# ShittyWizard/DiplomJourney

Hardware: AMD Instinct MI355X
Metric: candidate N-step rollouts/sec + MPC-step p50 latency, 1/2/4/8 MI355X (higher is better)
Workload: dtype f64

## Files before the change

diplomjourney_amd/csrc/mpc_device.h:

```cpp
#pragma once

#include <hip/hip_runtime.h>
#include <stdint.h>

#include "../../include/mpc_rollout.h"
#include "mpc_trig.h"

namespace mpc {

struct Consts {
  double x, y, phi;
  double x_t, y_t;
  double x_0, y_0;
  double A, B, C1, C2;
  double inv_den;
  double L, inv_L;
  double h;
  double hlgth;
  double s0, c0;
  int32_t L_pow2;
  int32_t pad_;
};

MPC_HD __forceinline__ Consts consts_from_problem(const mpc_problem_t& p) {
  Consts K;
  K.x = p.x;
  K.y = p.y;
  K.phi = p.phi;
  K.x_t = p.x_t;
  K.y_t = p.y_t;
  K.x_0 = p.x_0;
  K.y_0 = p.y_0;
  K.A = p.y_t - p.y_0;
  K.B = p.x_t - p.x_0;
  K.C1 = p.x_t * p.y_0;
  K.C2 = p.y_t * p.x_0;
  K.inv_den = 1.0 / sqrt(K.A * K.A + K.B * K.B);
  K.L = p.L;
  int e;
  const double m = frexp(p.L, &e);
  K.L_pow2 = (m == 0.5) ? 1 : 0;
  K.inv_L = K.L_pow2 ? 1.0 / p.L : 0.0;
  K.h = p.t_b - p.t_a;
  K.hlgth = 0.5 * (p.t_b - p.t_a);
  trig::sincos_fast(p.phi, &K.s0, &K.c0);
  K.pad_ = 0;
  return K;
}

constexpr double kWGK[11] = {
    0.011694638867371874278064396062192, 0.032558162307964727478818972459390,
    0.054755896574351996031381300244580, 0.075039674810919952767043140916190,
    0.093125454583697605535065465083366, 0.109387158802297641899210590325805,
    0.123491976262065851077208698889469, 0.134709217311473325928054001771707,
    0.142775938577060080797094273138717, 0.147739104901338491374841515972068,
    0.149445554002916905664936468389821};

template <int INTEG>
MPC_HD __forceinline__ double quad_const(double f, const Consts& K) {
  if constexpr (INTEG == MPC_INTEG_RECT) {
    return f * K.h;
  } else {
    double resk = kWGK[10] * f;
    const double fsum = f + f;
#pragma unroll
    for (int j = 1; j <= 9; j += 2) resk = resk + kWGK[j] * fsum;
#pragma unroll
    for (int j = 0; j <= 8; j += 2) resk = resk + kWGK[j] * fsum;
    return resk * K.hlgth;
  }
}

template <int INTEG>
MPC_HD __forceinline__ double heading_incr(double w, double t, const Consts& K) {
  if constexpr (INTEG == MPC_INTEG_RECT)
    return (w * K.h) * t;
  else
    return quad_const<INTEG>(w * t, K);
}

template <int INTEG>
MPC_HD __forceinline__ double position_step(double p, double v, double trig, const Consts& K) {
  if constexpr (INTEG == MPC_INTEG_RECT)
    return fma(v * K.h, trig, p);
  else
    return p + quad_const<INTEG>(v * trig, K);
}

constexpr int kRotCum = 2;

template <int INTEG, int ROT, bool PL2>
MPC_HD __forceinline__ void step_core(double& x, double& y, double& ph, double& s, double& c,
                                      double v, double beta, const Consts& K, bool& bad,
                                      const trig::Leads* ld = nullptr) {
  bad |= !(fabs(beta) <= trig::kTanMax);
  const double t = trig::tan_small(beta, ld);
  double dphi, vh = 0.0;
  if constexpr (PL2 && INTEG == MPC_INTEG_RECT && ROT == kRotCum) {
    vh = v * (K.h * K.inv_L);
    dphi = vh * t;
  } else if constexpr (PL2 && INTEG == MPC_INTEG_RECT) {
    vh = v * K.h;
    dphi = (vh * K.inv_L) * t;
  } else {
    const double w = PL2 ? v * K.inv_L : v / K.L;
    dphi = heading_incr<INTEG>(w, t, K);
  }
  ph = ph + dphi;
  if constexpr (ROT) {
    bad |= !(fabs(dphi) <= trig::kRotMax);
    double sd, cd;
    trig::rotation_sc(dphi, sd, cd, ld);
    trig::rotate_sc(sd, cd, s, c);
  } else {
    bad |= !(fabs(ph) <= trig::kFastMax);
    trig::sincos_core(ph, &s, &c);
  }
  if constexpr (PL2 && INTEG == MPC_INTEG_RECT) {
    x = fma(vh, c, x);
    y = fma(vh, s, y);
  } else {
    x = position_step<INTEG>(x, v, c, K);
    y = position_step<INTEG>(y, v, s, K);
  }
}

template <int ROT>
MPC_HD __forceinline__ void step_start(const Consts& K, double& x, double& y, double& ph,
                                       double& s, double& c) {
  ph = K.phi;
  if constexpr (ROT == kRotCum) {
    x = 0.0;
    y = 0.0;
    s = 0.0;
    c = 1.0;
  } else {
    x = K.x;
    y = K.y;
    s = K.s0;
    c = K.c0;
  }
}

template <bool SCALED>
MPC_HD __forceinline__ void cum_pose(const Consts& K, double A, double B, double& x, double& y) {
  if constexpr (SCALED) {
    A = A * K.L;
    B = B * K.L;
  }
  x = K.x + fma(K.c0, A, -(K.s0 * B));
  y = K.y + fma(K.s0, A, K.c0 * B);
}

template <int INTEG>
MPC_HD __forceinline__ void step_safe(double& x, double& y, double& ph, double v, double beta,
                                      const Consts& K) {
  const double w = K.L_pow2 ? v * K.inv_L : v / K.L;
  const double dphi = heading_incr<INTEG>(w, trig::tan_fast(beta), K);
  ph = ph + dphi;
  double s, c;
  trig::sincos_fast(ph, &s, &c);
  x = position_step<INTEG>(x, v, c, K);
  y = position_step<INTEG>(y, v, s, K);
}

MPC_HD __forceinline__ double crit_sqrt(double x) {
#if defined(__HIP_DEVICE_COMPILE__)
  const double y = __builtin_amdgcn_rsq(fmax(x, 0x1p-767));
  double g = x * y, h = y * 0.5;
  const double r = fma(-h, g, 0.5);
  g = fma(g, r, g);
  h = fma(h, r, h);
  double d = fma(-g, g, x);
  g = fma(d, h, g);
  d = fma(-g, g, x);
  return fma(d, h, g);
#else
  return sqrt(x);
#endif
}

MPC_HD __forceinline__ double cost(double x, double y, const Consts& K) {
  const double ex = K.x_t - x, ey = K.y_t - y;
  const double dist_target = crit_sqrt(ex * ex + ey * ey);
  const double dl = fabs(K.A * x - K.B * y + K.C1 - K.C2) * K.inv_den;
  const double d = (x == K.x_0 && y == K.y_0) ? 1000.0 : dl;
  return 10000.0 * dist_target + 10000.0 * (d * d);
}

struct Circle {
  double cx, cy, r2, pad_;
};
struct Obstacles {
  Circle c[MPC_MAX_OBSTACLES];
};
struct ObstacleArgs {
  Obstacles loop, world;
};
#if defined(__HIP_DEVICE_COMPILE__)
typedef const __attribute__((address_space(4))) Obstacles* ObsTable;
#else
typedef const Obstacles* ObsTable;
#endif

struct NoObs {
  static constexpr bool kOn = false;
};

template <int NOBS>
struct CircleObs {
  static_assert(NOBS >= 1 && NOBS <= MPC_MAX_OBSTACLES, "circle count");
  static constexpr bool kOn = true;
  ObsTable loop_t, world_t;
  template <int CPL>
  __device__ __forceinline__ static void test(ObsTable t, const double (&x)[CPL],
                                              const double (&y)[CPL], bool (&blocked)[CPL]) {
#if defined(__HIP_DEVICE_COMPILE__)
    if constexpr (NOBS > 4) asm volatile("" : "+s"(t));
#endif
#pragma unroll
    for (int i = 0; i < NOBS; ++i) {
      const double cx = t->c[i].cx, cy = t->c[i].cy, r2 = t->c[i].r2;
#pragma unroll
      for (int j = 0; j < CPL; ++j) {
        const double dx = x[j] - cx, dy = y[j] - cy;
        blocked[j] |= fma(dy, dy, dx * dx) < r2;
      }
    }
  }
  template <int CPL>
  __device__ __forceinline__ void loop(const double (&x)[CPL], const double (&y)[CPL],
                                       bool (&blocked)[CPL]) const {
    test<CPL>(loop_t, x, y, blocked);
  }
  __device__ __forceinline__ void world(double x, double y, bool& blocked) const {
    const double xs[1] = {x}, ys[1] = {y};
    bool bl[1] = {blocked};
    test<1>(world_t, xs, ys, bl);
    blocked = bl[0];
  }
};

MPC_HD __forceinline__ Circle frame_circle(const Consts& K, const Circle& w, bool scaled) {
  const double sc = scaled ? K.inv_L : 1.0;
  const double dx = w.cx - K.x, dy = w.cy - K.y;
  return Circle{(K.c0 * dx + K.s0 * dy) * sc, (K.c0 * dy - K.s0 * dx) * sc, w.r2 * (sc * sc), 0.0};
}

template <int INTEG, int ROT, bool PL2>
MPC_HD inline double rollout_candidate_l(const Consts& K, const double* v, const double* b,
                                         int64_t ld, int64_t col, int n_steps, double* traj) {
  double x, y, ph, s, c;
  step_start<ROT>(K, x, y, ph, s, c);
  bool bad = false;
  for (int st = 0; st < n_steps; ++st) {
    step_core<INTEG, ROT, PL2>(x, y, ph, s, c, v[st * ld + col], b[st * ld + col], K, bad);
    if (traj) {
      if constexpr (ROT == kRotCum) {
        cum_pose<PL2>(K, x, y, traj[3 * st + 0], traj[3 * st + 1]);
      } else {
        traj[3 * st + 0] = x;
        traj[3 * st + 1] = y;
      }
      traj[3 * st + 2] = ph;
    }
  }
  if constexpr (ROT == kRotCum) {
    if (!bad) cum_pose<PL2>(K, x, y, x, y);
  }
  if (bad) {
    x = K.x;
    y = K.y;
    ph = K.phi;
    for (int st = 0; st < n_steps; ++st) {
      step_safe<INTEG>(x, y, ph, v[st * ld + col], b[st * ld + col], K);
      if (traj) {
        traj[3 * st + 0] = x;
        traj[3 * st + 1] = y;
        traj[3 * st + 2] = ph;
      }
    }
  }
  return cost(x, y, K);
}

template <int INTEG, int ROT>
MPC_HD inline double rollout_candidate(const Consts& K, const double* v, const double* b,
                                       int64_t ld, int64_t col, int n_steps, double* traj) {
  return K.L_pow2 ? rollout_candidate_l<INTEG, ROT, true>(K, v, b, ld, col, n_steps, traj)
                  : rollout_candidate_l<INTEG, ROT, false>(K, v, b, ld, col, n_steps, traj);
}

}
```

diplomjourney_amd/csrc/mpc_generated.h:

```cpp
#pragma once

#include <hip/hip_runtime.h>
#include <stdint.h>

#include "mpc_argmin.h"
#include "mpc_device.h"
#include "mpc_episode.h"
#include "mpc_sampler.h"

namespace mpc {

__device__ inline void episode_grids(const mpc_episode_config_t& c, const EpisodeHead& S,
                                     double* s_v, double* s_b, int& nv_out, int& nb_out) {
  const int lane = threadIdx.x & 63;
  const uint64_t below = (lane == 0) ? 0ull : (~0ull >> (64 - lane));
  const int n_v = 1 + 2 * static_cast<int>(c.ratio_v);
  int nv = 0;
  double vmin = __builtin_inf();
  for (int base = 0; base < n_v; base += 64) {
    const int i = base + lane;
    const double cand = S.v + c.delta_v * (static_cast<double>(i) - c.ratio_v);
    const bool ok = i < n_v && !(cand < 0.0) && cand < c.v_max;
    const uint64_t m = __ballot(ok);
    const int pos = nv + __popcll(m & below);
    if (ok && pos < kEpMaxGrid) s_v[pos] = cand;
    if (S.steps_for_slowing > 0) {
      double mn = ok ? cand : __builtin_inf();
      for (int off = 32; off > 0; off >>= 1) mn = fmin(mn, __shfl_xor(mn, off, 64));
      vmin = fmin(vmin, mn);
    }
    nv += __popcll(m);
  }
  nv = nv < kEpMaxGrid ? nv : kEpMaxGrid;
  if (S.steps_for_slowing > 0 && nv > 0) {
    const double vel = vmin > c.v_min ? vmin : c.v_min;
    for (int i = lane; i < nv; i += 64) s_v[i] = vel;
  }
  const int n_b = 1 + 2 * static_cast<int>(c.ratio_beta);
  int nb = 0;
  for (int base = 0; base < n_b; base += 64) {
    const int i = base + lane;
    const double cand = S.beta + c.delta_beta * (static_cast<double>(i) - c.ratio_beta);
    const bool ok = i < n_b && fabs(cand) <= c.beta_bound;
    const uint64_t m = __ballot(ok);
    const int pos = nb + __popcll(m & below);
    if (ok && pos < kEpMaxGrid) s_b[pos] = cand;
    nb += __popcll(m);
  }
  nv_out = nv;
  nb_out = nb < kEpMaxGrid ? nb : kEpMaxGrid;
}

#ifndef MPC_TEMPLATES_ONLY
__global__ __launch_bounds__(kBlock) void k_episode_sample(
    mpc_episode_config_t c, EpisodeState* __restrict__ S, int64_t n_cand, int n_steps,
    int64_t base, double* __restrict__ v, double* __restrict__ b, int pairs) {
  __shared__ double s_v[kEpMaxGrid], s_b[kEpMaxGrid];
  __shared__ double2 s_grid[kSampleLdsEntries];
  __shared__ int s_nv, s_nb;
  if (threadIdx.x < 64) {
    int nv, nb;
    episode_grids(c, S->h, s_v, s_b, nv, nb);
    if (threadIdx.x == 0) {
      s_nv = nv;
      s_nb = nb;
    }
  }
  __syncthreads();
  const int nv = s_nv, nb = s_nb;
  const uint64_t seed = S->h.seed;
  const uint32_t n_grid = static_cast<uint32_t>(nv) * static_cast<uint32_t>(nb);
  const bool staged = n_grid <= static_cast<uint32_t>(kSampleLdsEntries);
  if (staged)
    for (uint32_t k = threadIdx.x; k < n_grid; k += kBlock)
      s_grid[k] = make_double2(s_v[k / nb], s_b[k % nb]);
  __syncthreads();
  if (blockIdx.x == 0 && threadIdx.x == 0) {
    S->h.nv = nv;
    S->h.nb = nb;
    for (int i = 0; i < nv; ++i) S->grid_v[i] = s_v[i];
    for (int i = 0; i < nb; ++i) S->grid_b[i] = s_b[i];
  }
  if (n_grid == 0 && !c.enumerate) return;
  if (!staged) {
    for (int64_t cc = blockIdx.x * static_cast<int64_t>(kBlock) + threadIdx.x; cc < n_cand;
         cc += static_cast<int64_t>(gridDim.x) * kBlock) {
      const uint64_t g = static_cast<uint64_t>(base + cc);
      for (int st = 0; st < n_steps; ++st) {
        const bool pad = c.enumerate && g >= n_grid;
        const uint32_t k = pad ? 0u : grid_entry(seed, st, g, n_grid, 1);
        v[ctl_off<false>(st, cc, n_cand)] = pad ? __builtin_nan("") : s_v[k / nb];
        b[ctl_off<false>(st, cc, n_cand)] = pad ? 0.0 : s_b[k % nb];
      }
    }
    return;
  }
  sample_items(s_grid, n_grid, n_cand, n_steps, seed, base, c.enumerate ? 2 : 1, v, b, n_cand,
               pairs);
}
#endif

template <int INTEG, int ROT, bool PL2>
__device__ __forceinline__ void generated_lane(const Consts& K, const double2* s_grid,
                                               uint32_t n_grid, uint64_t seed, uint64_t g0,
                                               int n_steps, double (&cst)[2]) {
  double x[2], y[2], ph[2], sn[2], cs[2];
  bool bad[2];
#pragma unroll
  for (int j = 0; j < 2; ++j) {
    step_start<ROT>(K, x[j], y[j], ph[j], sn[j], cs[j]);
    bad[j] = false;
  }
  trig::Leads lead = trig::const_leads();
#pragma unroll 1
  for (int st = 0; st < n_steps; ++st) {
    const double2 e0 = s_grid[grid_entry(seed, st, g0, n_grid, 1)];
    const double2 e1 = s_grid[grid_entry(seed, st, g0 + 1, n_grid, 1)];
    double ph0 = ROT ? 0.0 : ph[0], ph1 = ROT ? 0.0 : ph[1];
    step_core<INTEG, ROT, PL2>(x[0], y[0], ph0, sn[0], cs[0], e0.x, e0.y, K, bad[0], &lead);
    step_core<INTEG, ROT, PL2>(x[1], y[1], ph1, sn[1], cs[1], e1.x, e1.y, K, bad[1], &lead);
    if (!ROT) {
      ph[0] = ph0;
      ph[1] = ph1;
    }
  }
  if constexpr (ROT == kRotCum) {
#pragma unroll
    for (int j = 0; j < 2; ++j)
      if (!bad[j]) cum_pose<PL2>(K, x[j], y[j], x[j], y[j]);
  }
#pragma unroll
  for (int j = 0; j < 2; ++j) {
    if (bad[j]) {
      x[j] = K.x;
      y[j] = K.y;
      ph[j] = K.phi;
      for (int sr = 0; sr < n_steps; ++sr) {
        const double2 e = s_grid[grid_entry(seed, sr, g0 + j, n_grid, 1)];
        step_safe<INTEG>(x[j], y[j], ph[j], e.x, e.y, K);
      }
    }
    cst[j] = cost(x[j], y[j], K);
  }
}

constexpr int kGenWaves = 4;
template <int INTEG, int ROT, bool PL2>
__global__ __launch_bounds__(kBlock, kGenWaves) void k_rollout_generated(
    mpc_episode_config_t c, EpisodeState* __restrict__ S, int64_t n_cand, int n_steps,
    int64_t base, Rec* __restrict__ part, double* __restrict__ part_v,
    double* __restrict__ part_b) {
  extern __shared__ double2 s_gen_grid[];
  __shared__ double s_v[kEpMaxGrid], s_b[kEpMaxGrid];
  __shared__ int s_nv, s_nb;
  if (threadIdx.x < 64) {
    int nv, nb;
    episode_grids(c, S->h, s_v, s_b, nv, nb);
    if (threadIdx.x == 0) {
      s_nv = nv;
      s_nb = nb;
    }
  }
  __syncthreads();
  const int nv = s_nv, nb = s_nb;
  const uint32_t n_grid = static_cast<uint32_t>(nv) * static_cast<uint32_t>(nb);
  for (uint32_t k = threadIdx.x; k < n_grid; k += kBlock)
    s_gen_grid[k] = make_double2(s_v[k / nb], s_b[k % nb]);
  if (blockIdx.x == 0 && threadIdx.x == 0) {
    if ((S->h.K.L_pow2 != 0) != PL2) S->chain_error = 2u;
    S->h.nv = nv;
    S->h.nb = nb;
    for (int i = 0; i < nv; ++i) S->grid_v[i] = s_v[i];
    for (int i = 0; i < nb; ++i) S->grid_b[i] = s_b[i];
  }
  __syncthreads();
  const uint64_t seed = S->h.seed;
  const Consts K = S->h.K;
  const int64_t n_tiles = (n_cand + kBlock * 2 - 1) / (kBlock * 2);
  uint64_t best_k = ~0ull;
  int64_t best_i = INT64_MAX;
  if (n_grid > 0) {
    for (int64_t tile = blockIdx.x; tile < n_tiles; tile += gridDim.x) {
      const int64_t c0 = tile * (kBlock * 2) + threadIdx.x * 2;
      if (c0 < n_cand) {
        double cst[2];
        const uint64_t g0 = static_cast<uint64_t>(base + c0);
        generated_lane<INTEG, ROT, PL2>(K, s_gen_grid, n_grid, seed, g0, n_steps, cst);
#pragma unroll
        for (int j = 0; j < 2; ++j) {
          const uint64_t kk = cost_key_nonneg(cst[j]);
          if (kk < best_k) {
            best_k = kk;
            best_i = c0 + j;
          }
        }
      }
    }
  }
  block_argmin(best_k, best_i);
  if (threadIdx.x == 0) part[blockIdx.x] = Rec{best_k, best_i};
  __shared__ int64_t s_best;
  if (threadIdx.x == 0) s_best = best_k == ~0ull ? -1 : best_i;
  __syncthreads();
  const int64_t bi = s_best;
  if (bi >= 0 && threadIdx.x < n_steps) {
    const double2 e =
        s_gen_grid[grid_entry(seed, threadIdx.x, static_cast<uint64_t>(base + bi), n_grid, 1)];
    part_v[blockIdx.x * MPC_MAX_STEPS + threadIdx.x] = e.x;
    part_b[blockIdx.x * MPC_MAX_STEPS + threadIdx.x] = e.y;
  }
}

}
```

diplomjourney_amd/csrc/mpc_rollout.hip:

```cpp
#include <hip/hip_ext.h>
#include <hip/hip_runtime.h>

#include <math.h>
#include <stdint.h>
#include <string.h>

#include <algorithm>
#include <mutex>
#include <type_traits>

#include "../../include/mpc_rollout.h"
#include "mpc_argmin.h"
#include "mpc_chain.h"
#include "mpc_comm.h"
#include "mpc_device.h"
#include "mpc_dispatch.h"
#include "mpc_episode.h"
#include "mpc_episode_obs.h"
#include "mpc_episodes.h"
#include "mpc_episodes_obs_launch.h"
#include "mpc_exchange.h"
#include "mpc_finalize.h"
#include "mpc_ftepisodes.h"
#include "mpc_fulltree.h"
// ... 378 lines not shown
      k_episodes_run<I, R><<<n_robots, kBlock, 0, st>>>(dcfg, robots, n_steps, max_calls, log, cap,
                                                        progress);
    });
  else
    launch_episodes_run_obs(st, integrator, world_obstacles(obstacles, n_obstacles), n_obstacles,
                            n_robots, dcfg, robots, n_steps, max_calls, log, cap, progress,
                            n_blocked_out);
  return last_hip_status();
}

}
}

using namespace mpc;

extern "C" {

const char* mpc_version(void) { return "diplomjourney_amd mpc_rollout 0.2 (gfx950)"; }

const char* mpc_strerror(int status) {
  switch (status) {
    case MPC_OK: return "ok";
    case MPC_ERR_ARG: return "invalid argument";
    case MPC_ERR_WORKSPACE: return "workspace too small";
    case MPC_ERR_HIP: return "HIP runtime error";
    case MPC_ERR_UNSUPPORTED: return "unsupported option";
    default: return "unknown status";
  }
}

size_t mpc_workspace_bytes(int64_t n_cand, int32_t n_steps) {
  (void)n_steps;
  if (n_cand < 0) return 0;
  return static_cast<size_t>(rollout_blocks(n_cand)) * sizeof(Rec);
}

static int check_args(const mpc_problem_t* p, const double* v_sc, const double* beta_sc,
                      int64_t n_cand, int32_t n_steps, int32_t integrator, void* ws,
                      size_t ws_bytes) {
  if (!p || n_cand < 1 || n_steps < 1 || n_steps > MPC_MAX_STEPS || !v_sc || !beta_sc)
    return MPC_ERR_ARG;
  if (mode_ok(integrator) != MPC_OK) return MPC_ERR_UNSUPPORTED;
  if (!workspace_ok(ws, ws_bytes, n_cand, n_steps)) return MPC_ERR_WORKSPACE;
  return MPC_OK;
}

int mpc_rollout_partials(const mpc_problem_t* p, const double* v_sc, const double* beta_sc,
                         int64_t n_cand, int32_t n_steps, int32_t integrator, double* states_out,
                         void* ws, size_t ws_bytes, mpc_stream_t stream) {
  const int a = check_args(p, v_sc, beta_sc, n_cand, n_steps, integrator, ws, ws_bytes);
  if (a != MPC_OK) return a;
  hipStream_t st = reinterpret_cast<hipStream_t>(stream);
  const Consts K = host_consts(*p);
  Rec* part = static_cast<Rec*>(ws);
  if (states_out) {
    dispatch_mode(integrator, [&](auto I, auto R) {
      k_rollout_argmin<1, I, R, true, false>
          <<<rollout_grid<1>(n_cand), kBlock, 0, st>>>(
              K, nullptr, v_sc, beta_sc, n_cand, n_steps, part, states_out);
    });
  } else {
    launch_rollout<false>(st, integrator, K, nullptr, v_sc, beta_sc, n_cand, n_steps, part);
  }
  return last_hip_status();
}

int mpc_rollout_finalize(const mpc_problem_t* p, const double* v_sc, const double* beta_sc,
                         int64_t n_cand, int32_t n_steps, int64_t index_base, double incumbent,
                         int32_t integrator, int32_t with_states, void* ws, size_t ws_bytes,
                         mpc_result_t* out, mpc_stream_t stream) {
  const int a = check_args(p, v_sc, beta_sc, n_cand, n_steps, integrator, ws, ws_bytes);
  if (a != MPC_OK) return a;
  if (!out || index_base < 0) return MPC_ERR_ARG;
  const Consts K = host_consts(*p);
  const int n_part = static_cast<int>(partial_count(v_sc, beta_sc, n_cand, with_states != 0));
  launch_finalize<false>(reinterpret_cast<hipStream_t>(stream), integrator,
                         static_cast<const Rec*>(ws), n_part, K, nullptr, v_sc, beta_sc, n_cand,
                         n_steps, index_base, incumbent, nullptr, out, mpc_episode_config_t{},
                         EpisodeHook{});
  return last_hip_status();
}

int mpc_rollout_argmin(const mpc_problem_t* p, const double* v_sc, const double* beta_sc,
                       int64_t n_cand, int32_t n_steps, int64_t index_base, double incumbent,
                       int32_t integrator, double* states_out, void* ws, size_t ws_bytes,
                       mpc_result_t* out, mpc_stream_t stream) {
  if (!out || index_base < 0) return MPC_ERR_ARG;
  const int a = mpc_rollout_partials(p, v_sc, beta_sc, n_cand, n_steps, integrator, states_out,
                                     ws, ws_bytes, stream);
  if (a != MPC_OK) return a;
  return mpc_rollout_finalize(p, v_sc, beta_sc, n_cand, n_steps, index_base, incumbent,
                              integrator, states_out != nullptr, ws, ws_bytes, out, stream);
}

int mpc_rollout_partials_obstacles(const mpc_problem_t* p, const mpc_obstacle_t* obstacles,
                                   int32_t n_obstacles, const double* v_sc,
                                   const double* beta_sc, int64_t n_cand, int32_t n_steps,
                                   int32_t integrator, double* states_out, void* ws,
                                   size_t ws_bytes, int64_t* n_blocked_out, mpc_stream_t stream) {
  const int a = check_args(p, v_sc, beta_sc, n_cand, n_steps, integrator, ws, ws_bytes);
  if (a != MPC_OK) return a;
  const int o = check_obstacles(obstacles, n_obstacles);
  if (o != MPC_OK) return o;
  hipStream_t st = reinterpret_cast<hipStream_t>(stream);
  if (n_blocked_out &&
      hipMemsetAsync(n_blocked_out, 0, sizeof(*n_blocked_out), st) != hipSuccess)
    return MPC_ERR_HIP;
  if (n_obstacles == 0)
    return mpc_rollout_partials(p, v_sc, beta_sc, n_cand, n_steps, integrator, states_out, ws,
                                ws_bytes, stream);
  const Consts K = host_consts(*p);
  const ObstacleArgs O = host_obstacles(K, obstacles, n_obstacles, is_cum(integrator));
  launch_rollout_obs(st, integrator, K, O, n_obstacles, v_sc, beta_sc, n_cand, n_steps,
                     static_cast<Rec*>(ws), states_out,
                     reinterpret_cast<unsigned long long*>(n_blocked_out));
  return last_hip_status();
}

int mpc_rollout_argmin_obstacles(const mpc_problem_t* p, const mpc_obstacle_t* obstacles,
                                 int32_t n_obstacles, const double* v_sc, const double* beta_sc,
                                 int64_t n_cand, int32_t n_steps, int64_t index_base,
                                 double incumbent, int32_t integrator, double* states_out,
                                 void* ws, size_t ws_bytes, int64_t* n_blocked_out,
                                 mpc_result_t* out, mpc_stream_t stream) {
  if (!out || index_base < 0) return MPC_ERR_ARG;
  const int a = mpc_rollout_partials_obstacles(p, obstacles, n_obstacles, v_sc, beta_sc, n_cand,
                                               n_steps, integrator, states_out, ws, ws_bytes,
                                               n_blocked_out, stream);
  if (a != MPC_OK) return a;
  return mpc_rollout_finalize(p, v_sc, beta_sc, n_cand, n_steps, index_base, incumbent,
                              integrator, states_out != nullptr, ws, ws_bytes, out, stream);
}

size_t mpc_batched_workspace_bytes(int32_t n_problems, int64_t cand_per_problem, int32_t n_steps) {
  (void)n_steps;
  if (n_problems < 0 || cand_per_problem < 0) return 0;
  return static_cast<size_t>(n_problems) * static_cast<size_t>(rollout_blocks(cand_per_problem)) *
         sizeof(Rec);
}

int mpc_rollout_argmin_batched(const mpc_problem_t* problems, const double* incumbents,
                               int32_t n_problems, const double* v_sc, const double* beta_sc,
                               int64_t cand_per_problem, int32_t n_steps, int32_t integrator,
                               void* ws, size_t ws_bytes, mpc_result_t* out, mpc_stream_t stream) {
  if (!problems || !out || !v_sc || !beta_sc || n_problems < 1 || n_problems > 65535 ||
      cand_per_problem < 1 || n_steps < 1 || n_steps > MPC_MAX_STEPS)
    return MPC_ERR_ARG;
  if (mode_ok(integrator) != MPC_OK) return MPC_ERR_UNSUPPORTED;
  if (!ws || ws_bytes < mpc_batched_workspace_bytes(n_problems, cand_per_problem, n_steps))
    return MPC_ERR_WORKSPACE;
  hipStream_t st = reinterpret_cast<hipStream_t>(stream);
  const int64_t ld = static_cast<int64_t>(n_problems) * cand_per_problem;
  const bool wide = wide_ok(v_sc, beta_sc, cand_per_problem, ld);
  const int64_t tiles = cdiv(cand_per_problem, kBlock * (wide ? kCplWide : 1));
  const int64_t per_robot = std::min<int64_t>(tiles, rollout_blocks(cand_per_problem));
  const dim3 grid(static_cast<unsigned>(per_robot), static_cast<unsigned>(n_problems));
  Rec* part = static_cast<Rec*>(ws);
  dispatch_mode(integrator, [&](auto I, auto R) {
    if (wide)
      k_rollout_argmin_batched<kCplWide, I, R>
          <<<grid, kBlock, 0, st>>>(problems, v_sc, beta_sc, cand_per_problem, n_steps, ld, part);
    else
      k_rollout_argmin_batched<1, I, R>
          <<<grid, kBlock, 0, st>>>(problems, v_sc, beta_sc, cand_per_problem, n_steps, ld, part);
  });
  if (last_hip_status() != MPC_OK) return MPC_ERR_HIP;
  dispatch_mode(integrator, [&](auto I, auto R) {
    k_finalize_batched<I, R><<<n_problems, kBlock, 0, st>>>(
        part, static_cast<int>(per_robot), problems, incumbents, v_sc, beta_sc, cand_per_problem,
        n_steps, ld, out);
  });
  return last_hip_status();
}

int mpc_stream_probe(const double* v_sc, const double* beta_sc, int64_t n_cand,
                     int32_t n_steps, void* sink, size_t sink_bytes, mpc_stream_t stream) {
  if (!v_sc || !beta_sc || n_cand < 2 || n_steps < 1 || n_steps > MPC_MAX_STEPS || !sink)
    return MPC_ERR_ARG;
  if (!wide_ok(v_sc, beta_sc, n_cand)) return MPC_ERR_UNSUPPORTED;
  const int64_t grid = rollout_grid<kCplWide>(n_cand);
  if (sink_bytes < static_cast<size_t>(kMaxBlocks) * kBlock * sizeof(uint64_t))
    return MPC_ERR_WORKSPACE;
  k_stream_probe<false><<<grid, kBlock, 0, reinterpret_cast<hipStream_t>(stream)>>>(
      v_sc, beta_sc, n_cand, n_steps, static_cast<uint64_t*>(sink));
  return last_hip_status();
}

int mpc_stream_probe_tiled(const double* tiles, int64_t n_cand, int32_t n_steps, void* sink,
                           size_t sink_bytes, mpc_stream_t stream) {
  if (!tiles || n_steps < 1 || n_steps > MPC_MAX_STEPS || !sink) return MPC_ERR_ARG;
  if (!tiled_ok(tiles, tiles + MPC_TILE, n_cand)) return MPC_ERR_UNSUPPORTED;
  if (sink_bytes < static_cast<size_t>(kMaxBlocks) * kBlock * sizeof(uint64_t))
    return MPC_ERR_WORKSPACE;
  k_stream_probe<true><<<rollout_grid<kCplWide>(n_cand), kBlock, 0,
                         reinterpret_cast<hipStream_t>(stream)>>>(
      tiles, tiles + MPC_TILE, n_cand, n_steps, static_cast<uint64_t*>(sink));
  return last_hip_status();
}

__global__ void k_rcp_estimate(const double* __restrict__ q, double* __restrict__ r, int64_t n) {
  const int64_t i = static_cast<int64_t>(blockIdx.x) * blockDim.x + threadIdx.x;
  if (i < n) r[i] = trig::rcp_estimate(q[i]);
}

int mpc_rcp_estimate(const double* q, double* r, int64_t n, mpc_stream_t stream) {
  if (n < 0 || (n > 0 && (!q || !r))) return MPC_ERR_ARG;
  if (n == 0) return MPC_OK;
  k_rcp_estimate<<<static_cast<unsigned>(cdiv(n, kBlock)), kBlock, 0,
                   reinterpret_cast<hipStream_t>(stream)>>>(q, r, n);
  return last_hip_status();
}

int mpc_select_winner(const mpc_result_t* results, int32_t n, double incumbent,
                      mpc_result_t* out, mpc_stream_t stream) {
  if (!results || !out || n < 1) return MPC_ERR_ARG;
  k_select_winner<<<1, 64, 0, reinterpret_cast<hipStream_t>(stream)>>>(results, n, incumbent, out);
  return last_hip_status();
}

int mpc_sample_controls(const double* v_grid, int32_t n_v, const double* beta_grid,
                        int32_t n_beta, int64_t n_cand, int32_t n_steps, uint64_t seed,
                        int64_t index_base, int32_t const_prefix, double* v_sc,
                        double* beta_sc, int64_t ld, mpc_stream_t stream) {
  if (!v_grid || !beta_grid || !v_sc || !beta_sc || n_v < 1 || n_beta < 1 || n_cand < 1 ||
      n_steps < 1 || index_base < 0 || ld < n_cand)
    return MPC_ERR_ARG;
  if (static_cast<int64_t>(n_v) * n_beta > 0xFFFFFFFFll) return MPC_ERR_ARG;
  const int pairs = (n_cand % 2 == 0) && (ld % 2 == 0) && aligned16(v_sc) && aligned16(beta_sc);
  const int64_t items = pairs ? n_cand / 2 : n_cand;
  const int64_t grid = std::min<int64_t>(cdiv(items, kBlock), 4096);
  k_sample_controls<<<grid, kBlock, 0, reinterpret_cast<hipStream_t>(stream)>>>(
      v_grid, n_v, beta_grid, n_beta, n_cand, n_steps, seed, index_base, const_prefix, v_sc,
      beta_sc, ld, pairs, 0);
  return last_hip_status();
}

int mpc_sample_controls_tiled(const double* v_grid, int32_t n_v, const double* beta_grid,
                              int32_t n_beta, int64_t n_cand, int32_t n_steps, uint64_t seed,
                              int64_t index_base, int32_t const_prefix, double* tiles,
                              mpc_stream_t stream) {
  if (!v_grid || !beta_grid || !tiles || n_v < 1 || n_beta < 1 || n_steps < 1 ||
      n_steps > MPC_MAX_STEPS || index_base < 0)
    return MPC_ERR_ARG;
  if (static_cast<int64_t>(n_v) * n_beta > 0xFFFFFFFFll) return MPC_ERR_ARG;
  if (!tiled_ok(tiles, tiles + MPC_TILE, n_cand)) return MPC_ERR_ARG;
  const int64_t n_pad = cdiv(n_cand, MPC_TILE) * MPC_TILE;
  const int64_t grid = std::min<int64_t>(cdiv(n_pad / 2, kBlock), 4096);
  k_sample_controls<<<grid, kBlock, 0, reinterpret_cast<hipStream_t>(stream)>>>(
      v_grid, n_v, beta_grid, n_beta, n_pad, n_steps, seed, index_base, const_prefix, tiles,
      tiles + MPC_TILE, n_steps, 1, 1);
  return last_hip_status();
}

size_t mpc_episode_state_bytes(void) { return sizeof(EpisodeState); }

int mpc_episode_reset(const mpc_episode_config_t* cfg, void* state, mpc_stream_t stream) {
  if (check_episode_cfg(cfg) != MPC_OK || !state) return MPC_ERR_ARG;
  k_episode_reset<<<1, 64, 0, reinterpret_cast<hipStream_t>(stream)>>>(
      *cfg, static_cast<EpisodeState*>(state));
  return last_hip_status();
}

int mpc_episode_sample(const mpc_episode_config_t* cfg, void* state, double* v_sc,
                       double* beta_sc, int64_t n_cand, int32_t n_steps, int64_t index_base,
                       mpc_stream_t stream) {
  if (check_episode_cfg(cfg) != MPC_OK ||
      check_episode_arrays(state, v_sc, beta_sc, n_cand, n_steps) != MPC_OK || index_base < 0)
    return MPC_ERR_ARG;
  const int pairs = (n_cand % 2 == 0) && aligned16(v_sc) && aligned16(beta_sc);
  const int64_t items = pairs ? n_cand / 2 : n_cand;
  k_episode_sample<<<std::min<int64_t>(cdiv(items, kBlock), 4096), kBlock, 0,
                     reinterpret_cast<hipStream_t>(stream)>>>(
      *cfg, static_cast<EpisodeState*>(state), n_cand, n_steps, index_base, v_sc, beta_sc, pairs);
  return last_hip_status();
}

static int64_t gen_grid(int64_t n_cand) { return rollout_grid<2>(n_cand); }
static size_t gen_ctl_offset(int64_t n_cand) {
  return (static_cast<size_t>(gen_grid(n_cand)) * sizeof(Rec) + 255) & ~static_cast<size_t>(255);
}

size_t mpc_episode_generate_workspace_bytes(int64_t n_cand, int32_t n_steps) {
  (void)n_steps;
  if (n_cand < 2) return 0;
  return gen_ctl_offset(n_cand) +
         2 * static_cast<size_t>(gen_grid(n_cand)) * MPC_MAX_STEPS * sizeof(double);
}

int mpc_episode_generate_step(const mpc_episode_config_t* cfg, void* state, int64_t n_cand,
                              int32_t n_steps, int64_t index_base, int32_t integrator, void* ws,
                              size_t ws_bytes, mpc_result_t* out, mpc_episode_log_t* log,
                              int32_t log_capacity, mpc_stream_t stream) {
  if (check_episode_cfg(cfg) != MPC_OK || !state || !out || n_steps < 1 ||
      n_steps > MPC_MAX_STEPS || index_base < 0 || log_capacity < 0)
    return MPC_ERR_ARG;
  if (n_cand < 2 || n_cand % 2 != 0) return MPC_ERR_ARG;
  if (mode_ok(integrator) != MPC_OK || cfg->enumerate) return MPC_ERR_UNSUPPORTED;
  if (!ws || ws_bytes < mpc_episode_generate_workspace_bytes(n_cand, n_steps))
    return MPC_ERR_WORKSPACE;
  static_assert(kEpMaxGrid * kEpMaxGrid * sizeof(double2) <= 64 * 1024, "grid LDS bound");
  const int64_t nv = std::min<int64_t>(kEpMaxGrid, 1 + 2 * static_cast<int64_t>(cfg->ratio_v));
  const int64_t nb =
      std::min<int64_t>(kEpMaxGrid, 1 + 2 * static_cast<int64_t>(cfg->ratio_beta));
  const size_t lds = static_cast<size_t>(nv * nb) * sizeof(double2);
  EpisodeState* S = static_cast<EpisodeState*>(state);
  hipStream_t st = reinterpret_cast<hipStream_t>(stream);
  char* w = static_cast<char*>(ws);
  Rec* part = reinterpret_cast<Rec*>(w);
  const int64_t grid = gen_grid(n_cand);
  double* part_v = reinterpret_cast<double*>(w + gen_ctl_offset(n_cand));
  double* part_b = part_v + grid * MPC_MAX_STEPS;
  const EpisodeHook hook = episode_hook(S, true, log, log_capacity);
  bool launched = true;
  dispatch_mode(integrator, [&](auto I, auto R) {
    dispatch_bools(
        [&](auto PL2) {
          if (lds > 48 * 1024)
            launched = hipFuncSetAttribute(
                           reinterpret_cast<const void*>(&k_rollout_generated<I, R, PL2>),
                           hipFuncAttributeMaxDynamicSharedMemorySize,
                           static_cast<int>(lds)) == hipSuccess;
          if (launched) {
            k_rollout_generated<I, R, PL2><<<grid, kBlock, lds, st>>>(
                *cfg, S, n_cand, n_steps, index_base, part, part_v, part_b);
            launched = hipPeekAtLastError() == hipSuccess;
          }
        },
        length_pow2(cfg->L));
    if (launched)
      k_finalize_gen<I, R><<<1, kFinBlock, 0, st>>>(part, static_cast<int>(grid), &S->h.K, part_v,
                                                    part_b, n_steps, index_base, &S->h.incumbent,
                                                    out, *cfg, hook);
  });
  if (!launched) {
    (void)hipGetLastError();
    return MPC_ERR_HIP;
  }
  return last_hip_status();
}

int mpc_episode_partials(void* state, const double* v_sc, const double* beta_sc, int64_t n_cand,
                         int32_t n_steps, int32_t integrator, void* ws, size_t ws_bytes,
                         mpc_stream_t stream) {
  return episode_partials(state, nullptr, 0, v_sc, beta_sc, n_cand, n_steps, integrator, ws,
                          ws_bytes, nullptr, stream);
}

int mpc_episode_finalize(void* state, const double* v_sc, const double* beta_sc, int64_t n_cand,
                         int32_t n_steps, int64_t index_base, int32_t integrator, void* ws,
                         size_t ws_bytes, mpc_result_t* out, const mpc_episode_config_t* advance,
                         mpc_episode_log_t* log, int32_t log_capacity, mpc_stream_t stream) {
  const int a = check_episode_finish(state, v_sc, beta_sc, n_cand, n_steps, index_base, integrator,
                                     true, ws, ws_bytes, out, advance, log_capacity);
  if (a != MPC_OK) return a;
  EpisodeState* S = static_cast<EpisodeState*>(state);
  const int n_part = static_cast<int>(is_tiled(integrator)
                                          ? rollout_grid<kCplWide>(n_cand)
                                          : partial_count(v_sc, beta_sc, n_cand, false));
  launch_finalize<true>(reinterpret_cast<hipStream_t>(stream), integrator,
                        static_cast<const Rec*>(ws), n_part, Consts{}, &S->h.K, v_sc, beta_sc,
                        n_cand, n_steps, index_base, 0.0, &S->h.incumbent, out,
                        advance ? *advance : mpc_episode_config_t{},
                        episode_hook(S, advance != nullptr, log, log_capacity));
  return last_hip_status();
}

int mpc_episode_step(void* state, const double* v_sc, const double* beta_sc, int64_t n_cand,
                     int32_t n_steps, int64_t index_base, int32_t integrator, void* ws,
                     size_t ws_bytes, mpc_result_t* out, const mpc_episode_config_t* advance,
                     mpc_episode_log_t* log, int32_t log_capacity, mpc_stream_t stream) {
  const int a =
      mpc_episode_partials(state, v_sc, beta_sc, n_cand, n_steps, integrator, ws, ws_bytes, stream);
  if (a != MPC_OK) return a;
  return mpc_episode_finalize(state, v_sc, beta_sc, n_cand, n_steps, index_base, integrator, ws,
                              ws_bytes, out, advance, log, log_capacity, stream);
}

int mpc_episode_partials_obstacles(void* state, const mpc_obstacle_t* obstacles,
                                   int32_t n_obstacles, const double* v_sc,
                                   const double* beta_sc, int64_t n_cand, int32_t n_steps,
                                   int32_t integrator, void* ws, size_t ws_bytes,
                                   int64_t* n_blocked_out, mpc_stream_t stream) {
  return episode_partials(state, obstacles, n_obstacles, v_sc, beta_sc, n_cand, n_steps,
                          integrator, ws, ws_bytes, n_blocked_out, stream);
}

int mpc_episode_step_obstacles(void* state, const mpc_obstacle_t* obstacles, int32_t n_obstacles,
                               const double* v_sc, const double* beta_sc, int64_t n_cand,
                               int32_t n_steps, int64_t index_base, int32_t integrator, void* ws,
                               size_t ws_bytes, mpc_result_t* out,
                               const mpc_episode_config_t* advance, mpc_episode_log_t* log,
                               int32_t log_capacity, int64_t* n_blocked_out,
                               mpc_stream_t stream) {
  const int a = mpc_episode_partials_obstacles(state, obstacles, n_obstacles, v_sc, beta_sc, n_cand,
                                               n_steps, integrator, ws, ws_bytes, n_blocked_out,
                                               stream);
  if (a != MPC_OK) return a;
  return mpc_episode_finalize(state, v_sc, beta_sc, n_cand, n_steps, index_base, integrator, ws,
                              ws_bytes, out, advance, log, log_capacity, stream);
}

int mpc_episode_rollout(void* state, const double* v_sc, const double* beta_sc, int64_t n_cand,
                        int32_t n_steps, int64_t index_base, int32_t integrator, void* ws,
                        size_t ws_bytes, mpc_result_t* out, const mpc_episode_config_t* advance,
                        mpc_episode_log_t* log, int32_t log_capacity, mpc_stream_t stream) {
  const int a = check_episode_finish(state, v_sc, beta_sc, n_cand, n_steps, index_base, integrator,
                                     false, ws, ws_bytes, out, advance, log_capacity);
  if (a != MPC_OK) return a;
  EpisodeState* S = static_cast<EpisodeState*>(state);
  const mpc_episode_config_t ecfg = advance ? *advance : mpc_episode_config_t{};
  const EpisodeHook hook = episode_hook(S, advance != nullptr, log, log_capacity);
  hipStream_t st = reinterpret_cast<hipStream_t>(stream);
  const bool wide = wide_ok(v_sc, beta_sc, n_cand);
  dispatch_mode(integrator, [&](auto I, auto R) {
    if (wide)
      k_rollout_episode<kCplWide, I, R><<<fused_grid<kCplWide, I, R>(n_cand), kBlock, 0, st>>>(
          &S->h.K, v_sc, beta_sc, n_cand, n_steps, index_base, static_cast<Rec*>(ws), &S->done,
          &S->h.incumbent, out, ecfg, hook);
    else
      k_rollout_episode<1, I, R><<<fused_grid<1, I, R>(n_cand), kBlock, 0, st>>>(
          &S->h.K, v_sc, beta_sc, n_cand, n_steps, index_base, static_cast<Rec*>(ws), &S->done,
          &S->h.incumbent, out, ecfg, hook);
  });
  return last_hip_status();
}

int mpc_episode_chain_step(const mpc_episode_config_t* cfg, void* state, int32_t mode,
                           uint32_t epoch, const double* v_sc, const double* beta_sc,
                           int64_t n_cand, int32_t n_steps, int64_t index_base,
                           int32_t integrator, void* ws, const void* ws_prev, size_t ws_bytes,
                           const double* v_prev, const double* beta_prev, mpc_result_t* out_prev,
                           const mpc_result_t* , int32_t ,
                           mpc_episode_log_t* log, int32_t log_capacity, mpc_stream_t stream) {
  return episode_chain_step(cfg, state, nullptr, 0, mode, epoch, v_sc, beta_sc, n_cand, n_steps,
                            index_base, integrator, ws, ws_prev, ws_bytes, v_prev, beta_prev,
                            out_prev, log, log_capacity, nullptr, stream);
}

int mpc_episode_chain_step_obstacles(
    const mpc_episode_config_t* cfg, void* state, const mpc_obstacle_t* obstacles,
    int32_t n_obstacles, int32_t mode, uint32_t epoch, const double* v_sc, const double* beta_sc,
    int64_t n_cand, int32_t n_steps, int64_t index_base, int32_t integrator, void* ws,
    const void* ws_prev, size_t ws_bytes, const double* v_prev, const double* beta_prev,
    mpc_result_t* out_prev, const mpc_result_t* , int32_t ,
    mpc_episode_log_t* log, int32_t log_capacity, int64_t* n_blocked_out, mpc_stream_t stream) {
  return episode_chain_step(cfg, state, obstacles, n_obstacles, mode, epoch, v_sc, beta_sc, n_cand,
                            n_steps, index_base, integrator, ws, ws_prev, ws_bytes, v_prev,
                            beta_prev, out_prev, log, log_capacity, n_blocked_out, stream);
}

#ifdef MPC_RUN_STATS
int mpc_debug_run_stats(unsigned long long* host, int reset) {
  if (reset) {
    unsigned long long init[kRunMaxSteps][8];
    for (int j = 0; j < kRunMaxSteps; ++j)
      for (int f = 0; f < 8; ++f) init[j][f] = (f == 3) ? ~0ull : 0ull;
    return hipMemcpyToSymbol(HIP_SYMBOL(g_run_tl), init, sizeof(init)) == hipSuccess ? 0 : -1;
  }
  return hipMemcpyFromSymbol(host, HIP_SYMBOL(g_run_tl), sizeof(g_run_tl)) == hipSuccess ? 0 : -1;
}
#endif

size_t mpc_episode_run_workspace_bytes(int64_t n_cand) {
  if (n_cand < 2) return 0;
  return run_workspace_bytes(cdiv(n_cand, kBlock * kCplWide));
}

int mpc_episode_run(const mpc_episode_config_t* cfg, void* state, uint32_t epoch0,
                    const double* const* v_steps, const double* const* beta_steps, int32_t n_run,
                    int64_t n_cand, int32_t n_steps, int64_t index_base, int32_t integrator,
                    void* ws, size_t ws_bytes, mpc_result_t* out, mpc_episode_log_t* log,
                    int32_t log_capacity, mpc_stream_t stream) {
  if (!chained_args_ok(cfg, state, v_steps, beta_steps, n_cand, n_steps, index_base, log_capacity,
                       epoch0) ||
      n_cand < 2 || n_run < 1 || !out)
    return MPC_ERR_ARG;
  if (static_cast<uint64_t>(epoch0) + static_cast<uint64_t>(n_run) - 1u > 0xFFFFFFFFull)
    return MPC_ERR_ARG;
  if (n_cand > 0x7fffffffll) return MPC_ERR_ARG;
  if (!chained_mode_ok(integrator, true)) return MPC_ERR_UNSUPPORTED;
  for (int32_t j = 0; j < n_run; ++j)
    if (!v_steps[j] || !beta_steps[j] || !chain_ctl_ok(v_steps[j], beta_steps[j], n_cand, integrator))
      return MPC_ERR_UNSUPPORTED;
  if (!ws || ws_bytes < mpc_episode_run_workspace_bytes(n_cand)) return MPC_ERR_WORKSPACE;
  if (!wall_clock_ok()) return MPC_ERR_UNSUPPORTED;
  EpisodeState* S = static_cast<EpisodeState*>(state);
  hipStream_t st = reinterpret_cast<hipStream_t>(stream);
  const int64_t tiles = cdiv(n_cand, kBlock * kCplWide);
  for (int32_t j0 = 0; j0 < n_run; j0 += kRunMaxSteps) {
    const int k = std::min<int32_t>(kRunMaxSteps, n_run - j0);
    RunArgs ra;
    memset(&ra, 0, sizeof(ra));
    for (int j = 0; j < k; ++j) {
      ra.ctl.v[j] = v_steps[j0 + j];
      ra.ctl.b[j] = beta_steps[j0 + j];
    }
    ra.S = S;
    ra.ws = ws;
    ra.out = out;
    ra.log = log;
    ra.n_cand = n_cand;
    ra.index_base = index_base;
    ra.e0 = epoch0 + static_cast<uint32_t>(j0);
    ra.K = k;
    ra.n_steps = n_steps;
    ra.T = static_cast<int>(tiles);
    ra.cap = log_capacity;
    ra.ecfg = *cfg;
    dispatch_bools(
        [&](auto PL2, auto TILED) {
          const int64_t grid = 1 + run_tile_blocks<PL2, TILED>(tiles * k);
          k_episode_run<PL2, TILED><<<grid, kBlock, 0, st>>>(ra);
        },
        length_pow2(cfg->L), is_tiled(integrator));
    if (hipPeekAtLastError() != hipSuccess) break;
  }
  return last_hip_status();
}

int mpc_episode_exchange_step(const mpc_episode_config_t* cfg, void* state, uint32_t epoch,
                              const double* v_sc, const double* beta_sc, int64_t n_cand,
                              int32_t n_steps, int64_t index_base, int32_t integrator, void* ws,
                              size_t ws_bytes, const mpc_candidate_t* gathered,
                              int32_t n_gathered, mpc_result_t* out_prev, mpc_candidate_t* local,
                              mpc_episode_log_t* log, int32_t log_capacity, mpc_stream_t stream) {
  return mpc_episode_exchange_step2(cfg, state, epoch, 0u, v_sc, beta_sc, n_cand, n_steps,
                                    index_base, integrator, ws, ws_bytes, gathered, n_gathered,
                                    out_prev, local, log, log_capacity, stream);
}

int mpc_episode_exchange_step2(const mpc_episode_config_t* cfg, void* state, uint32_t epoch,
                               uint32_t wait_tag, const double* v_sc, const double* beta_sc,
                               int64_t n_cand, int32_t n_steps, int64_t index_base,
                               int32_t integrator, void* ws, size_t ws_bytes,
                               const mpc_candidate_t* gathered, int32_t n_gathered,
                               mpc_result_t* out_prev, mpc_candidate_t* local,
                               mpc_episode_log_t* log, int32_t log_capacity,
                               mpc_stream_t stream) {
  if (!chained_args_ok(cfg, state, v_sc, beta_sc, n_cand, n_steps, index_base, log_capacity,
                       epoch) ||
      !local || !out_prev)
    return MPC_ERR_ARG;
  if (n_cand > 0x7fffffffll || (gathered && n_gathered < 1)) return MPC_ERR_ARG;
  if (wait_tag && (!gathered || n_gathered > kXchgLdsRanks)) return MPC_ERR_ARG;
  if (!chained_mode_ok(integrator, false) || !wide_ok(v_sc, beta_sc, n_cand))
    return MPC_ERR_UNSUPPORTED;
  if (!workspace_ok(ws, ws_bytes, n_cand, n_steps)) return MPC_ERR_WORKSPACE;
  if (!wall_clock_ok()) return MPC_ERR_UNSUPPORTED;
  EpisodeState* S = static_cast<EpisodeState*>(state);
  const int64_t grid = rollout_grid<kCplWide>(n_cand) + 1;
  hipStream_t st = reinterpret_cast<hipStream_t>(stream);
  dispatch_bools(
      [&](auto PL2) {
        k_episode_chain<MPC_INTEG_RECT, kRotCum, kChainXchg, PL2><<<grid, kBlock, 0, st>>>(
            S, epoch, v_sc, beta_sc, n_cand, n_steps, static_cast<Rec*>(ws), gathered ? 1 : 0,
            reinterpret_cast<const Rec*>(local), 0, nullptr, nullptr, index_base, out_prev,
            gathered, n_gathered, *cfg, log, log_capacity, gathered ? wait_tag : 0u);
      },
      length_pow2(cfg->L));
  return last_hip_status();
}

int mpc_stream_create_cu_reserved(int32_t reserved_per_xcd, mpc_stream_t* stream) {
  if (!stream || reserved_per_xcd < 0 || reserved_per_xcd > 8) return MPC_ERR_ARG;
  int dev = 0, ncu = 0;
  hipDeviceProp_t prop;
  if (hipGetDevice(&dev) != hipSuccess ||
      hipDeviceGetAttribute(&ncu, hipDeviceAttributeMultiprocessorCount, dev) != hipSuccess ||
      hipGetDeviceProperties(&prop, dev) != hipSuccess)
    return MPC_ERR_HIP;
  if (ncu != 256 || strncmp(prop.gcnArchName, "gfx950", 6) != 0)
    return MPC_ERR_UNSUPPORTED;
  uint32_t mask[16];
  const int words = (ncu + 31) / 32;
  if (words > 16) return MPC_ERR_UNSUPPORTED;
  for (int w = 0; w < words; ++w) mask[w] = 0xffffffffu;
  for (int b = 0; b < 8 * reserved_per_xcd; ++b) mask[b / 32] &= ~(1u << (b % 32));
  hipStream_t st = nullptr;
  if (hipExtStreamCreateWithCUMask(&st, static_cast<uint32_t>(words), mask) != hipSuccess)
    return MPC_ERR_HIP;
  *stream = reinterpret_cast<mpc_stream_t>(st);
  return MPC_OK;
}

int mpc_stream_create_cu_share(int32_t part, int32_t parts, mpc_stream_t* stream) {
  if (!stream || parts < 1 || parts > 32 || part < 0 || part >= parts) return MPC_ERR_ARG;
  int dev = 0, ncu = 0;
  hipDeviceProp_t prop;
  if (hipGetDevice(&dev) != hipSuccess ||
      hipDeviceGetAttribute(&ncu, hipDeviceAttributeMultiprocessorCount, dev) != hipSuccess ||
      hipGetDeviceProperties(&prop, dev) != hipSuccess)
    return MPC_ERR_HIP;
  if (ncu != 256 || strncmp(prop.gcnArchName, "gfx950", 6) != 0) return MPC_ERR_UNSUPPORTED;
  uint32_t mask[8] = {};
  for (int b = 0; b < ncu; ++b)
    if ((b / 8) % parts == part) mask[b / 32] |= 1u << (b % 32);
  hipStream_t st = nullptr;
  if (hipExtStreamCreateWithCUMask(&st, 8u, mask) != hipSuccess) return MPC_ERR_HIP;
  *stream = reinterpret_cast<mpc_stream_t>(st);
  return MPC_OK;
}

int mpc_stream_destroy(mpc_stream_t stream) {
  if (!stream) return MPC_ERR_ARG;
  return hipStreamDestroy(reinterpret_cast<hipStream_t>(stream)) == hipSuccess ? MPC_OK
                                                                               : MPC_ERR_HIP;
}

int mpc_episode_exchange_mark(void* state, uint32_t tag, mpc_stream_t stream) {
  if (!state || tag == 0) return MPC_ERR_ARG;
  k_exchange_mark<<<1, 64, 0, reinterpret_cast<hipStream_t>(stream)>>>(
      static_cast<EpisodeState*>(state), tag);
  return last_hip_status();
}

int mpc_episode_exchange_flush(const mpc_episode_config_t* cfg, void* state, int32_t integrator,
                               const mpc_candidate_t* gathered, int32_t n_gathered,
                               mpc_result_t* out, mpc_episode_log_t* log, int32_t log_capacity,
                               mpc_stream_t stream) {
  if (check_episode_cfg(cfg) != MPC_OK || !state || !gathered || n_gathered < 1 || !out ||
      log_capacity < 0)
    return MPC_ERR_ARG;
  if (mode_ok(integrator) != MPC_OK || !is_cum(integrator)) return MPC_ERR_UNSUPPORTED;
  k_episode_advance_cand<MPC_INTEG_RECT, kRotCum>
      <<<1, kFinBlock, 0, reinterpret_cast<hipStream_t>(stream)>>>(
          *cfg, static_cast<EpisodeState*>(state), gathered, n_gathered, out, log, log_capacity);
  return last_hip_status();
}

size_t mpc_mailbox_bytes(int32_t world) {
  return world < 1 || world > kMailMaxRanks ? 0 : mailbox_bytes(world);
// ... 469 lines not shown
```

Baseline: 33.11 billion.

## Precompute per-grid-entry step factors into an LDS table for generated rollouts

For small control grids, each block now precomputes per-(v,beta) step factors (tan, rotation sin/cos, position scale, bad flag) into a shared-memory table. The rollout loop then looks these up instead of recomputing tan and rotation trig every step. Table loads are software-pipelined one step ahead, and the occupancy target rises to 6 waves for the rotation path. The cost is a larger LDS footprint per entry (32 vs 16 bytes), extra kernel instantiations, and a recompute fallback path for bad rollouts.

```diff
diff --git a/diplomjourney_amd/csrc/mpc_device.h b/diplomjourney_amd/csrc/mpc_device.h
--- a/diplomjourney_amd/csrc/mpc_device.h
+++ b/diplomjourney_amd/csrc/mpc_device.h
@@ -125,6 +125,64 @@
   }
 }
 
+struct StepFactors {
+  double pf, sd, cd, dphi;
+  bool bad;
+};
+
+template <int INTEG, int ROT, bool PL2>
+MPC_HD __forceinline__ StepFactors step_factors(double v, double beta, const Consts& K,
+                                                const trig::Leads* ld = nullptr) {
+  StepFactors f;
+  f.bad = !(fabs(beta) <= trig::kTanMax);
+  const double t = trig::tan_small(beta, ld);
+  double dphi, vh = 0.0;
+  if constexpr (PL2 && INTEG == MPC_INTEG_RECT && ROT == kRotCum) {
+    vh = v * (K.h * K.inv_L);
+    dphi = vh * t;
+  } else if constexpr (PL2 && INTEG == MPC_INTEG_RECT) {
+    vh = v * K.h;
+    dphi = (vh * K.inv_L) * t;
+  } else {
+    const double w = PL2 ? v * K.inv_L : v / K.L;
+    dphi = heading_incr<INTEG>(w, t, K);
+  }
+  f.dphi = dphi;
+  f.sd = 0.0;
+  f.cd = 0.0;
+  if constexpr (ROT) {
+    f.bad |= !(fabs(dphi) <= trig::kRotMax);
+    trig::rotation_sc(dphi, f.sd, f.cd, ld);
+  }
+  if constexpr (PL2 && INTEG == MPC_INTEG_RECT)
+    f.pf = vh;
+  else if constexpr (INTEG == MPC_INTEG_RECT)
+    f.pf = v * K.h;
+  else
+    f.pf = v;
+  return f;
+}
+
+template <int INTEG, int ROT, bool PL2>
+MPC_HD __forceinline__ void step_apply(double& x, double& y, double& ph, double& s, double& c,
+                                       const StepFactors& f, const Consts& K, bool& bad) {
+  bad |= f.bad;
+  ph = ph + f.dphi;
+  if constexpr (ROT) {
+    trig::rotate_sc(f.sd, f.cd, s, c);
+  } else {
+    bad |= !(fabs(ph) <= trig::kFastMax);
+    trig::sincos_core(ph, &s, &c);
+  }
+  if constexpr (INTEG == MPC_INTEG_RECT) {
+    x = fma(f.pf, c, x);
+    y = fma(f.pf, s, y);
+  } else {
+    x = x + quad_const<INTEG>(f.pf * c, K);
+    y = y + quad_const<INTEG>(f.pf * s, K);
+  }
+}
+
 template <int ROT>
 MPC_HD __forceinline__ void step_start(const Consts& K, double& x, double& y, double& ph,
                                        double& s, double& c) {
diff --git a/diplomjourney_amd/csrc/mpc_generated.h b/diplomjourney_amd/csrc/mpc_generated.h
--- a/diplomjourney_amd/csrc/mpc_generated.h
+++ b/diplomjourney_amd/csrc/mpc_generated.h
@@ -144,13 +144,107 @@
   }
 }
 
+struct alignas(16) GenEntry {
+  double pf;
+  double a;
+  double cd;
+  uint32_t bad;
+  uint32_t pad_;
+};
+constexpr int kGenTableMax = 1025;
+
+template <int INTEG, int ROT, bool PL2>
+__device__ __forceinline__ GenEntry gen_entry(double v, double beta, const Consts& K) {
+  const StepFactors f = step_factors<INTEG, ROT, PL2>(v, beta, K);
+  return GenEntry{f.pf, ROT ? f.sd : f.dphi, f.cd, f.bad ? 1u : 0u, 0u};
+}
+
+__device__ __forceinline__ StepFactors gen_factors(const GenEntry& e, bool rot) {
+  return StepFactors{e.pf, rot ? e.a : 0.0, e.cd, rot ? 0.0 : e.a, false};
+}
+
+__device__ __forceinline__ uint32_t grid_entry_sel(uint64_t sg, int s, uint32_t n_grid, bool pre,
+                                                   uint32_t g32) {
+  const uint64_t h = splitmix64(sg ^ (static_cast<uint64_t>(s) << 40));
+  const uint32_t k = static_cast<uint32_t>(((h >> 32) * static_cast<uint64_t>(n_grid)) >> 32);
+  return pre ? g32 : k;
+}
+
+template <int INTEG, int ROT, bool PL2>
+__device__ __forceinline__ void generated_lane_tab(const Consts& K, const GenEntry* tab,
+                                                   const double* s_v, const double* s_b,
+                                                   uint32_t nb, uint32_t n_grid, uint64_t seed,
+                                                   uint64_t g0, int n_steps, double (&cst)[2]) {
+  double x[2], y[2], ph[2], sn[2], cs[2];
+  bool bad[2], pre[2];
+  uint64_t sg[2];
+  uint32_t g32[2], badw[2];
+  GenEntry e[2];
+#pragma unroll
+  for (int j = 0; j < 2; ++j) {
+    step_start<ROT>(K, x[j], y[j], ph[j], sn[j], cs[j]);
+    bad[j] = false;
+    badw[j] = 0u;
+    sg[j] = seed ^ (g0 + j);
+    pre[j] = g0 + j < n_grid;
+    g32[j] = static_cast<uint32_t>(g0 + j);
+    e[j] = tab[grid_entry_sel(sg[j], 0, n_grid, pre[j], g32[j])];
+  }
+  auto step = [&](int st) {
+    StepFactors f[2];
+#pragma unroll
+    for (int j = 0; j < 2; ++j) {
+      f[j] = gen_factors(e[j], ROT != 0);
+      badw[j] |= e[j].bad;
+      e[j] = tab[grid_entry_sel(sg[j], st + 1, n_grid, pre[j], g32[j])];
+    }
+#pragma unroll
+    for (int j = 0; j < 2; ++j) {
+      double phj = ROT ? 0.0 : ph[j];
+      step_apply<INTEG, ROT, PL2>(x[j], y[j], phj, sn[j], cs[j], f[j], K, bad[j]);
+      if (!ROT) ph[j] = phj;
+    }
+  };
+  if constexpr (ROT != 0) {
+#pragma unroll 2
+    for (int st = 0; st < n_steps; ++st) step(st);
+  } else {
+#pragma unroll 1
+    for (int st = 0; st < n_steps; ++st) step(st);
+  }
+#pragma unroll
+  for (int j = 0; j < 2; ++j) bad[j] |= badw[j] != 0u;
+  if constexpr (ROT == kRotCum) {
+#pragma unroll
+    for (int j = 0; j < 2; ++j)
+      if (!bad[j]) cum_pose<PL2>(K, x[j], y[j], x[j], y[j]);
+  }
+#pragma unroll
+  for (int j = 0; j < 2; ++j) {
+    if (bad[j]) {
+      x[j] = K.x;
+      y[j] = K.y;
+      ph[j] = K.phi;
+      for (int sr = 0; sr < n_steps; ++sr) {
+        const uint32_t k = grid_entry(seed, sr, g0 + j, n_grid, 1);
+        step_safe<INTEG>(x[j], y[j], ph[j], s_v[k / nb], s_b[k % nb], K);
+      }
+    }
+    cst[j] = cost(x[j], y[j], K);
+  }
+}
+
 constexpr int kGenWaves = 4;
-template <int INTEG, int ROT, bool PL2>
-__global__ __launch_bounds__(kBlock, kGenWaves) void k_rollout_generated(
+constexpr int kGenTabWaves = 6;
+template <int INTEG, int ROT, bool PL2, bool TAB>
+__global__ __launch_bounds__(kBlock, TAB && ROT ? kGenTabWaves : kGenWaves)
+void k_rollout_generated(
     mpc_episode_config_t c, EpisodeState* __restrict__ S, int64_t n_cand, int n_steps,
     int64_t base, Rec* __restrict__ part, double* __restrict__ part_v,
     double* __restrict__ part_b) {
-  extern __shared__ double2 s_gen_grid[];
+  extern __shared__ double2 s_gen_dyn[];
+  double2* const s_gen_grid = s_gen_dyn;
+  GenEntry* const s_tab = reinterpret_cast<GenEntry*>(s_gen_dyn);
   __shared__ double s_v[kEpMaxGrid], s_b[kEpMaxGrid];
   __shared__ int s_nv, s_nb;
   if (threadIdx.x < 64) {
@@ -164,8 +258,17 @@
   __syncthreads();
   const int nv = s_nv, nb = s_nb;
   const uint32_t n_grid = static_cast<uint32_t>(nv) * static_cast<uint32_t>(nb);
-  for (uint32_t k = threadIdx.x; k < n_grid; k += kBlock)
-    s_gen_grid[k] = make_double2(s_v[k / nb], s_b[k % nb]);
+  Consts K;
+  uint64_t seed;
+  if constexpr (TAB) {
+    K = S->h.K;
+    seed = S->h.seed;
+    for (uint32_t k = threadIdx.x; k < n_grid; k += kBlock)
+      s_tab[k] = gen_entry<INTEG, ROT, PL2>(s_v[k / nb], s_b[k % nb], K);
+  } else {
+    for (uint32_t k = threadIdx.x; k < n_grid; k += kBlock)
+      s_gen_grid[k] = make_double2(s_v[k / nb], s_b[k % nb]);
+  }
   if (blockIdx.x == 0 && threadIdx.x == 0) {
     if ((S->h.K.L_pow2 != 0) != PL2) S->chain_error = 2u;
     S->h.nv = nv;
@@ -174,8 +277,10 @@
     for (int i = 0; i < nb; ++i) S->grid_b[i] = s_b[i];
   }
   __syncthreads();
-  const uint64_t seed = S->h.seed;
-  const Consts K = S->h.K;
+  if constexpr (!TAB) {
+    seed = S->h.seed;
+    K = S->h.K;
+  }
   const int64_t n_tiles = (n_cand + kBlock * 2 - 1) / (kBlock * 2);
   uint64_t best_k = ~0ull;
   int64_t best_i = INT64_MAX;
@@ -185,7 +290,11 @@
       if (c0 < n_cand) {
         double cst[2];
         const uint64_t g0 = static_cast<uint64_t>(base + c0);
-        generated_lane<INTEG, ROT, PL2>(K, s_gen_grid, n_grid, seed, g0, n_steps, cst);
+        if constexpr (TAB)
+          generated_lane_tab<INTEG, ROT, PL2>(K, s_tab, s_v, s_b, static_cast<uint32_t>(nb),
+                                              n_grid, seed, g0, n_steps, cst);
+        else
+          generated_lane<INTEG, ROT, PL2>(K, s_gen_grid, n_grid, seed, g0, n_steps, cst);
 #pragma unroll
         for (int j = 0; j < 2; ++j) {
           const uint64_t kk = cost_key_nonneg(cst[j]);
@@ -204,8 +313,13 @@
   __syncthreads();
   const int64_t bi = s_best;
   if (bi >= 0 && threadIdx.x < n_steps) {
-    const double2 e =
-        s_gen_grid[grid_entry(seed, threadIdx.x, static_cast<uint64_t>(base + bi), n_grid, 1)];
+    const uint32_t k =
+        grid_entry(seed, threadIdx.x, static_cast<uint64_t>(base + bi), n_grid, 1);
+    double2 e;
+    if constexpr (TAB)
+      e = make_double2(s_v[k / nb], s_b[k % nb]);
+    else
+      e = s_gen_grid[k];
     part_v[blockIdx.x * MPC_MAX_STEPS + threadIdx.x] = e.x;
     part_b[blockIdx.x * MPC_MAX_STEPS + threadIdx.x] = e.y;
   }
diff --git a/diplomjourney_amd/csrc/mpc_rollout.hip b/diplomjourney_amd/csrc/mpc_rollout.hip
--- a/diplomjourney_amd/csrc/mpc_rollout.hip
+++ b/diplomjourney_amd/csrc/mpc_rollout.hip
@@ -704,7 +704,10 @@
   const int64_t nv = std::min<int64_t>(kEpMaxGrid, 1 + 2 * static_cast<int64_t>(cfg->ratio_v));
   const int64_t nb =
       std::min<int64_t>(kEpMaxGrid, 1 + 2 * static_cast<int64_t>(cfg->ratio_beta));
-  const size_t lds = static_cast<size_t>(nv * nb) * sizeof(double2);
+  static_assert(sizeof(GenEntry) == 32 && kGenTableMax * sizeof(GenEntry) <= 48 * 1024,
+                "table LDS bound");
+  const bool tab = nv * nb <= kGenTableMax;
+  const size_t lds = static_cast<size_t>(nv * nb) * (tab ? sizeof(GenEntry) : sizeof(double2));
   EpisodeState* S = static_cast<EpisodeState*>(state);
   hipStream_t st = reinterpret_cast<hipStream_t>(stream);
   char* w = static_cast<char*>(ws);
@@ -716,19 +719,19 @@
   bool launched = true;
   dispatch_mode(integrator, [&](auto I, auto R) {
     dispatch_bools(
-        [&](auto PL2) {
+        [&](auto PL2, auto TAB) {
           if (lds > 48 * 1024)
             launched = hipFuncSetAttribute(
-                           reinterpret_cast<const void*>(&k_rollout_generated<I, R, PL2>),
+                           reinterpret_cast<const void*>(&k_rollout_generated<I, R, PL2, TAB>),
                            hipFuncAttributeMaxDynamicSharedMemorySize,
                            static_cast<int>(lds)) == hipSuccess;
           if (launched) {
-            k_rollout_generated<I, R, PL2><<<grid, kBlock, lds, st>>>(
+            k_rollout_generated<I, R, PL2, TAB><<<grid, kBlock, lds, st>>>(
                 *cfg, S, n_cand, n_steps, index_base, part, part_v, part_b);
             launched = hipPeekAtLastError() == hipSuccess;
           }
         },
-        length_pow2(cfg->L));
+        length_pow2(cfg->L), tab);
     if (launched)
       k_finalize_gen<I, R><<<1, kFinBlock, 0, st>>>(part, static_cast<int>(grid), &S->h.K, part_v,
                                                     part_b, n_steps, index_base, &S->h.incumbent,
```

After: 32.80 billion. No clear change (-0.9%).
